# bjing2016/mdgen

Hardware: AMD Instinct MI355X
Metric: sampled MD frames/sec (higher is better)
Workload: dtype bf16; 1 GPU; tetrapeptide_fwdsim_crop4_T1000_B16; batch_per_gpu=16, num_frames=1000, crop=4, euler_steps=49, hipgraph=True, parallelism=batch-sharded x1, no collective

## Files before the change

mdgen_amd/csrc/k_rows.hip:

```cpp
#include "kernels.h"
#include "rows.h"

namespace mdg {

struct MlpPipe {
    f32x16 y[12];
    f32x16 a1[2][2];
    bf16x8 hf[2][4];
    bf16x8 wr[kWRing];
    f32x4 bias;
    float gx[4], gp[4], gq[4];
};

__device__ __forceinline__ void acc_rearm(f32x16& t, int r, float b) {
    float z;
    asm("v_accvgpr_write_b32 %0, %1" : "=a"(z) : "v"(b));
    t[r] = z;
}
constexpr float kGelu3C0 = -2.301208258e+00f, kGelu3C1 = -1.066924557e-01f, kGelu3C2 = 1.000115648e-03f;
template <int ST, bool REARM>
__device__ __forceinline__ void gelu_stage(MlpPipe& m, f32x16 (&a1r)[2], int g, bf16x8 (&hfw)[4]) {
    const int tile = g >> 2, a = g & 3;
    if (ST == 0) {
#pragma unroll
        for (int j = 0; j < 4; ++j) asm("v_accvgpr_read_b32 %0, %1" : "=v"(m.gx[j]) : "a"(a1r[tile][4 * a + j]));
    } else if (ST == 1) {
#pragma unroll
        for (int j = 0; j < 4; ++j) m.gq[j] = m.gx[j] * m.gx[j];
    } else if (ST == 2) {
#pragma unroll
        for (int j = 0; j < 4; ++j) m.gq[j] = fminf(m.gq[j], 64.0f);
    } else if (ST == 3) {
#pragma unroll
        for (int j = 0; j < 4; ++j) m.gp[j] = kGelu3C2 * m.gq[j] + kGelu3C1;
    } else if (ST == 4) {
#pragma unroll
        for (int j = 0; j < 4; ++j) m.gp[j] = m.gp[j] * m.gq[j] + kGelu3C0;
    } else if (ST == 5) {
#pragma unroll
        for (int j = 0; j < 4; ++j) m.gp[j] = m.gx[j] * m.gp[j];
    } else if (ST == 6) {
        m.gp[0] = __builtin_amdgcn_exp2f(m.gp[0]);
        m.gp[1] = __builtin_amdgcn_exp2f(m.gp[1]);
        if (REARM) {
            acc_rearm(a1r[tile], 4 * a + 0, m.bias[0]);
            acc_rearm(a1r[tile], 4 * a + 1, m.bias[1]);
        }
    } else if (ST == 7) {
        m.gp[2] = __builtin_amdgcn_exp2f(m.gp[2]);
        m.gp[3] = __builtin_amdgcn_exp2f(m.gp[3]);
        m.gp[0] = 1.0f + m.gp[0];
        m.gp[1] = 1.0f + m.gp[1];
    } else if (ST == 8) {
        m.gp[0] = __builtin_amdgcn_rcpf(m.gp[0]);
        m.gp[1] = __builtin_amdgcn_rcpf(m.gp[1]);
        m.gp[2] = 1.0f + m.gp[2];
        m.gp[3] = 1.0f + m.gp[3];
    } else if (ST == 9) {
        m.gp[2] = __builtin_amdgcn_rcpf(m.gp[2]);
        m.gp[3] = __builtin_amdgcn_rcpf(m.gp[3]);
        m.gx[0] = m.gx[0] * m.gp[0];
        m.gx[1] = m.gx[1] * m.gp[1];
    } else if (ST == 10) {
        m.gx[2] = m.gx[2] * m.gp[2];
        m.gx[3] = m.gx[3] * m.gp[3];
        if (REARM) {
            acc_rearm(a1r[tile], 4 * a + 2, m.bias[2]);
            acc_rearm(a1r[tile], 4 * a + 3, m.bias[3]);
        }
    } else {
        const int kk = 2 * tile + (a >> 1), e0 = 4 * (a & 1);
        hfw[kk][e0 + 0] = (__bf16)m.gx[0];
        hfw[kk][e0 + 1] = (__bf16)m.gx[1];
        hfw[kk][e0 + 2] = (__bf16)m.gx[2];
        hfw[kk][e0 + 3] = (__bf16)m.gx[3];
    }
}
template <bool REARM, int ST = 0>
__device__ __forceinline__ void gelu_stages_from(MlpPipe& m, f32x16 (&a1r)[2], int g, bf16x8 (&hfw)[4]) {
    gelu_stage<ST, REARM>(m, a1r, g, hfw);
    if constexpr (ST < 11) gelu_stages_from<REARM, ST + 1>(m, a1r, g, hfw);
}
__device__ __forceinline__ void rearm(f32x16 (&a1r)[2], int g, const f32x4& b) {
    const int tile = g >> 2, a = g & 3;
#pragma unroll
    for (int j = 0; j < 4; ++j) acc_rearm(a1r[tile], 4 * a + j, b[j]);
}
__device__ __forceinline__ void arm_chunk(f32x16 (&a1)[2], const float* b1c) {
#pragma unroll
    for (int g = 0; g < 8; ++g) rearm(a1, g, *reinterpret_cast<const f32x4*>(b1c + 32 * (g >> 2) + 8 * (g & 3)));
}

template <class WS, int D0, int STRIDE>
__device__ __forceinline__ void issue_q(const WS& ws, long slot, int q) {
    switch (q / STRIDE) {
        case 0: ws.template issue<D0 + 0>(slot); break;
        case 1: ws.template issue<D0 + 1>(slot); break;
        case 2: ws.template issue<D0 + 2>(slot); break;
        case 3: if constexpr (12 / STRIDE > 3) ws.template issue<D0 + 3>(slot); break;
        case 4: if constexpr (12 / STRIDE > 4) ws.template issue<D0 + 4>(slot); break;
        case 5: if constexpr (12 / STRIDE > 5) ws.template issue<D0 + 5>(slot); break;
        case 6: if constexpr (12 / STRIDE > 6) ws.template issue<D0 + 6>(slot); break;
        case 7: if constexpr (12 / STRIDE > 7) ws.template issue<D0 + 7>(slot); break;
        case 8: if constexpr (12 / STRIDE > 8) ws.template issue<D0 + 8>(slot); break;
        case 9: if constexpr (12 / STRIDE > 9) ws.template issue<D0 + 9>(slot); break;
        case 10: if constexpr (12 / STRIDE > 10) ws.template issue<D0 + 10>(slot); break;
        default: if constexpr (12 / STRIDE > 11) ws.template issue<D0 + 11>(slot); break;
    }
}

template <bool REARM>
__device__ __forceinline__ void gelu_stage_q(MlpPipe& m, f32x16 (&a1r)[2], int g, int q, bf16x8 (&hfw)[4]) {
    switch (q) {
        case 0: gelu_stage<0, REARM>(m, a1r, g, hfw); break;
        case 1: gelu_stage<1, REARM>(m, a1r, g, hfw); break;
        case 2: gelu_stage<2, REARM>(m, a1r, g, hfw); break;
        case 3: gelu_stage<3, REARM>(m, a1r, g, hfw); break;
        case 4: gelu_stage<4, REARM>(m, a1r, g, hfw); break;
        case 5: gelu_stage<5, REARM>(m, a1r, g, hfw); break;
        case 6: gelu_stage<6, REARM>(m, a1r, g, hfw); break;
        case 7: gelu_stage<7, REARM>(m, a1r, g, hfw); break;
        case 8: gelu_stage<8, REARM>(m, a1r, g, hfw); break;
        case 9: gelu_stage<9, REARM>(m, a1r, g, hfw); break;
        case 10: gelu_stage<10, REARM>(m, a1r, g, hfw); break;
        default: gelu_stage<11, REARM>(m, a1r, g, hfw); break;
    }
}

template <int NW, int I0, int KIND, int KI, int GG, bool REARM, int BARVM, bool FILL, int NLOOK = 12, class WS>
__device__ __forceinline__ void pipe_block(MlpPipe& m, const bf16x8 (&xf)[24], f32x16 (&a1w)[2], f32x16 (&a1r)[2],
                                           bf16x8 (&hfw)[4], const bf16x8 (&hfr)[4], const float* b1n,
                                           const unsigned char* ring_lane, const WS& ws, long fill_slot) {
    constexpr int FPW = WS::FPW, DPB = FPW / 2, STRIDE = 12 / DPB;
    if (BARVM >= 0) ring_barrier<BARVM>();
    __builtin_amdgcn_sched_barrier(0);
#pragma unroll
    for (int q = 0; q < 12; ++q) {
        const int I = I0 + q;
        if (FILL && q % STRIDE == 0) issue_q<WS, ((I0 / 12) & 1) * DPB, STRIDE>(ws, fill_slot, q);
        if (q < NLOOK) m.wr[(I + kWPF) % kWRing] = *reinterpret_cast<const bf16x8*>(ring_lane + ((I + kWPF) % kRingFrags) * 1024);
        if (GG >= 0 && REARM && q == 0) m.bias = *reinterpret_cast<const f32x4*>(b1n + 32 * (GG >> 2) + 8 * (GG & 3));
        if (KIND == 0) {
            const int ks = 6 * KI + (q >> 1), tile = q & 1;
            a1w[tile] = __builtin_amdgcn_mfma_f32_32x32x16_bf16(m.wr[I % kWRing], xf[ks], a1w[tile], 0, 0, 0);
        } else {
            m.y[q] = __builtin_amdgcn_mfma_f32_32x32x16_bf16(m.wr[I % kWRing], hfr[KI], m.y[q], 0, 0, 0);
        }
        if (GG >= 0) gelu_stage_q<REARM>(m, a1r, GG, q, hfw);
        __builtin_amdgcn_sched_barrier(0);
    }
}

template <bool REARM>
__device__ __forceinline__ void gelu_group_plain(MlpPipe& m, f32x16 (&a1r)[2], const float* b1n, int g, bf16x8 (&hfw)[4]) {
    if (REARM) m.bias = *reinterpret_cast<const f32x4*>(b1n + 32 * (g >> 2) + 8 * (g & 3));
    gelu_stages_from<REARM>(m, a1r, g, hfw);
}

#define ROWS_STAMP(i)                                  \
    st[i] = __builtin_amdgcn_s_memtime();              \
    __builtin_amdgcn_sched_barrier(0)

template <int NW, bool MODLDS, bool FOLD = false, bool TAIL = false>
__global__ __launch_bounds__(NW * 64, 1) void k_mlp_rows(const MlpRowsParams p) {
    static_assert(!FOLD || MODLDS, "the folded form: one modulation group per launch");
    static_assert(!TAIL || FOLD, "the tail runs on the folded form's accumulators");
    __shared__ __attribute__((aligned(1024))) unsigned char smem[kRingBytes + 8192 + NW * 6144 + (TAIL ? 4096 : 0)];
    using WS = WStream<NW>;
    constexpr int FPW = WS::FPW;
    const int w = __builtin_amdgcn_readfirstlane(wave_id()), lane = lane_id(), hh = lane >> 5, n = lane & 31;
    unsigned long long st[8] = {};
    ROWS_STAMP(0);
    WS ws{p.wstream, lds_addr(smem), (unsigned)lane * 16u, w};
#pragma unroll
    for (int i = 0; i < 6; ++i)
        if (i % NW == w)
            dma_frag<0, true>(reinterpret_cast<const unsigned char*>(p.b1) + i * 1024, (unsigned)lane * 16u,
                              lds_addr(smem) + kRingBytes + i * 1024);
    if (TAIL) {
#pragma unroll
        for (int c = 0; c < 2; ++c)
            if (c % NW == w) {
                const unsigned char* src = reinterpret_cast<const unsigned char*>(p.tail_mod) + c * (kC * 4);
                dma_frag<0, true>(src, (unsigned)lane * 16u, lds_addr(smem) + kRingBytes + 8192 + NW * 6144 + c * 2048);
                dma_frag<1024, false>(src, (unsigned)lane * 16u, lds_addr(smem) + kRingBytes + 8192 + NW * 6144 + c * 2048);
            }
    }
    const long t = ((long)blockIdx.x * NW + w) * 32 + n;
    const int tok = t < p.nrows ? (int)t : -1;
    float* modl = reinterpret_cast<float*>(smem + kRingBytes + 8192 + w * 6144);
    {
        if (MODLDS) {
            const long t0 = ((long)blockIdx.x * NW + w) * 32;
            const unsigned char* mb = reinterpret_cast<const unsigned char*>(p.mm.mod + p.mm.row_off(t0 < p.nrows ? t0 : 0));
            const int chunk[3] = {p.scale_chunk, p.shift_chunk, p.gate_chunk};
#pragma unroll
            for (int c = 0; c < 3; ++c) {
                const unsigned char* src = FOLD && c == 2 ? reinterpret_cast<const unsigned char*>(p.b2g) : mb + (long)chunk[c] * (kC * 4);
                dma_frag<0, true>(src, (unsigned)lane * 16u, lds_addr(modl) + c * 2048);
                dma_frag<1024, false>(src, (unsigned)lane * 16u, lds_addr(modl) + c * 2048);
            }
        }
    }
    ws.issue_slot(0);
    ws.issue_slot(1);
    ws.issue_slot(2);
    float* b1s = reinterpret_cast<float*>(smem + kRingBytes);
    bf16x8 xf[24];
    MlpPipe m;
    const unsigned char* ring_lane = smem + lane * 16;
    if (MODLDS) {
        f32x4 v[48];
        rows_load(p.h, tok, v);
        asm volatile("s_waitcnt vmcnt(0)" ::: "memory");
        if (FOLD) rows_norm_lds_fold(v, tok, modl, modl + 512, modl + 1024, 1e-6f, xf, m.y);
        else rows_norm_lds(v, tok, modl, modl + 512, 1e-6f, xf);
    } else {
        rows_ln(p.h, tok, p.mm, p.shift_chunk, p.scale_chunk, 1e-6f, xf);
    }
    ROWS_STAMP(1);
    if (!FOLD) rows_acc_init(m.y, p.b2);
    const float* b1l = b1s + 4 * hh;
    ring_barrier<FPW>();
#pragma unroll
    for (int i = 0; i < kWPF; ++i) m.wr[i] = *reinterpret_cast<const bf16x8*>(ring_lane + i * 1024);
    arm_chunk(m.a1[0], b1l);
    arm_chunk(m.a1[1], b1l + 64);
    pipe_block<NW, 0, 0, 0, -1, false, -1, true>(m, xf, m.a1[0], m.a1[1], m.hf[0], m.hf[1], b1l, ring_lane, ws, 3);
    pipe_block<NW, 12, 0, 1, -1, false, -1, true>(m, xf, m.a1[0], m.a1[1], m.hf[0], m.hf[1], b1l, ring_lane, ws, 3);
    pipe_block<NW, 24, 0, 2, -1, false, FPW, true>(m, xf, m.a1[0], m.a1[1], m.hf[0], m.hf[1], b1l, ring_lane, ws, 4);
    pipe_block<NW, 36, 0, 3, -1, false, -1, true>(m, xf, m.a1[0], m.a1[1], m.hf[0], m.hf[1], b1l, ring_lane, ws, 4);
    pipe_block<NW, 48, 0, 0, 0, true, FPW, true>(m, xf, m.a1[1], m.a1[0], m.hf[0], m.hf[1], b1l + 128, ring_lane, ws, 5);
    gelu_group_plain<true>(m, m.a1[0], b1l + 128, 1, m.hf[0]);
    pipe_block<NW, 60, 0, 1, 2, true, -1, true>(m, xf, m.a1[1], m.a1[0], m.hf[0], m.hf[1], b1l + 128, ring_lane, ws, 5);
    gelu_group_plain<true>(m, m.a1[0], b1l + 128, 3, m.hf[0]);
    pipe_block<NW, 72, 0, 2, 4, true, FPW, true>(m, xf, m.a1[1], m.a1[0], m.hf[0], m.hf[1], b1l + 128, ring_lane, ws, 6);
    gelu_group_plain<true>(m, m.a1[0], b1l + 128, 5, m.hf[0]);
    pipe_block<NW, 84, 0, 3, 6, true, -1, true>(m, xf, m.a1[1], m.a1[0], m.hf[0], m.hf[1], b1l + 128, ring_lane, ws, 6);
    gelu_group_plain<true>(m, m.a1[0], b1l + 128, 7, m.hf[0]);
    ROWS_STAMP(2);
#pragma unroll 1
    for (int c = 1; c < 23; c += 2) {
        {
            const long s0 = 4 * c;
            const float* bn = b1l + 64 * (c + 2);
            pipe_block<NW, 0, 0, 0, 0, true, FPW, true>(m, xf, m.a1[0], m.a1[1], m.hf[1], m.hf[0], bn, ring_lane, ws, s0 + 3);
            pipe_block<NW, 12, 1, 0, 1, true, -1, true>(m, xf, m.a1[0], m.a1[1], m.hf[1], m.hf[0], bn, ring_lane, ws, s0 + 3);
            pipe_block<NW, 24, 0, 1, 2, true, FPW, true>(m, xf, m.a1[0], m.a1[1], m.hf[1], m.hf[0], bn, ring_lane, ws, s0 + 4);
            pipe_block<NW, 36, 1, 1, 3, true, -1, true>(m, xf, m.a1[0], m.a1[1], m.hf[1], m.hf[0], bn, ring_lane, ws, s0 + 4);
            pipe_block<NW, 48, 0, 2, 4, true, FPW, true>(m, xf, m.a1[0], m.a1[1], m.hf[1], m.hf[0], bn, ring_lane, ws, s0 + 5);
            pipe_block<NW, 60, 1, 2, 5, true, -1, true>(m, xf, m.a1[0], m.a1[1], m.hf[1], m.hf[0], bn, ring_lane, ws, s0 + 5);
            pipe_block<NW, 72, 0, 3, 6, true, FPW, true>(m, xf, m.a1[0], m.a1[1], m.hf[1], m.hf[0], bn, ring_lane, ws, s0 + 6);
            pipe_block<NW, 84, 1, 3, 7, true, -1, true>(m, xf, m.a1[0], m.a1[1], m.hf[1], m.hf[0], bn, ring_lane, ws, s0 + 6);
        }
        {
            const long s0 = 4 * (c + 1);
            const float* bn = b1l + 64 * (c + 3);
            pipe_block<NW, 0, 0, 0, 0, true, FPW, true>(m, xf, m.a1[1], m.a1[0], m.hf[0], m.hf[1], bn, ring_lane, ws, s0 + 3);
            pipe_block<NW, 12, 1, 0, 1, true, -1, true>(m, xf, m.a1[1], m.a1[0], m.hf[0], m.hf[1], bn, ring_lane, ws, s0 + 3);
            pipe_block<NW, 24, 0, 1, 2, true, FPW, true>(m, xf, m.a1[1], m.a1[0], m.hf[0], m.hf[1], bn, ring_lane, ws, s0 + 4);
            pipe_block<NW, 36, 1, 1, 3, true, -1, true>(m, xf, m.a1[1], m.a1[0], m.hf[0], m.hf[1], bn, ring_lane, ws, s0 + 4);
            pipe_block<NW, 48, 0, 2, 4, true, FPW, true>(m, xf, m.a1[1], m.a1[0], m.hf[0], m.hf[1], bn, ring_lane, ws, s0 + 5);
            pipe_block<NW, 60, 1, 2, 5, true, -1, true>(m, xf, m.a1[1], m.a1[0], m.hf[0], m.hf[1], bn, ring_lane, ws, s0 + 5);
            pipe_block<NW, 72, 0, 3, 6, true, FPW, true>(m, xf, m.a1[1], m.a1[0], m.hf[0], m.hf[1], bn, ring_lane, ws, s0 + 6);
            pipe_block<NW, 84, 1, 3, 7, true, -1, true>(m, xf, m.a1[1], m.a1[0], m.hf[0], m.hf[1], bn, ring_lane, ws, s0 + 6);
        }
    }
    ROWS_STAMP(3);
    pipe_block<NW, 0, 1, 0, 0, false, FPW, true>(m, xf, m.a1[0], m.a1[1], m.hf[1], m.hf[0], b1l, ring_lane, ws, 95);
    gelu_group_plain<false>(m, m.a1[1], b1l, 1, m.hf[1]);
    pipe_block<NW, 12, 1, 1, 2, false, -1, true>(m, xf, m.a1[0], m.a1[1], m.hf[1], m.hf[0], b1l, ring_lane, ws, 95);
    gelu_group_plain<false>(m, m.a1[1], b1l, 3, m.hf[1]);
    pipe_block<NW, 24, 1, 2, 4, false, FPW, false>(m, xf, m.a1[0], m.a1[1], m.hf[1], m.hf[0], b1l, ring_lane, ws, 0);
    gelu_group_plain<false>(m, m.a1[1], b1l, 5, m.hf[1]);
    pipe_block<NW, 36, 1, 3, 6, false, -1, false>(m, xf, m.a1[0], m.a1[1], m.hf[1], m.hf[0], b1l, ring_lane, ws, 0);
    gelu_group_plain<false>(m, m.a1[1], b1l, 7, m.hf[1]);
    pipe_block<NW, 48, 1, 0, -1, false, 0, false>(m, xf, m.a1[0], m.a1[1], m.hf[0], m.hf[1], b1l, ring_lane, ws, 0);
    pipe_block<NW, 60, 1, 1, -1, false, -1, false>(m, xf, m.a1[0], m.a1[1], m.hf[0], m.hf[1], b1l, ring_lane, ws, 0);
    pipe_block<NW, 72, 1, 2, -1, false, 0, false>(m, xf, m.a1[0], m.a1[1], m.hf[0], m.hf[1], b1l, ring_lane, ws, 0);
    pipe_block<NW, 84, 1, 3, -1, false, -1, false, 12 - kWPF>(m, xf, m.a1[0], m.a1[1], m.hf[0], m.hf[1], b1l, ring_lane, ws, 0);
    ROWS_STAMP(4);
    if (TAIL) {
        const float* fmod = reinterpret_cast<const float*>(smem + kRingBytes + 8192 + NW * 6144);
        float xnew[16];
        rows_final_tail(m.y, tok, fmod + 512, fmod, p.tail_w, p.tail_b, p.tail_D, p.tail_euler, p.tail_dt, p.tail_x, p.tail_out, xf, xnew);
        ROWS_STAMP(6);
        if (p.emb_base) {
            rows_embed_tail(m.y, tok, xnew, EmbedTail{p.emb_wl_hi, p.emb_wl_lo, p.emb_wc_hi, p.emb_wc_lo, p.emb_base, p.emb_mdelta, p.emb_xcond, p.emb_cmask, p.emb_T, p.emb_L, p.tail_D});
            ROWS_STAMP(7);
            rows_write<0, 12>(m.y, tok, p.h);
        }
    } else if (FOLD) {
        rows_write<0, 12>(m.y, tok, p.h);
    } else if (MODLDS) {
        rows_gate_residual_lds<0, 6>(m.y, tok, modl + 1024, p.h);
        rows_gate_residual_lds<6, 12>(m.y, tok, modl + 1024, p.h);
    } else {
        rows_gate_residual<0, 6>(m.y, tok, p.mm, p.gate_chunk, p.h);
        rows_gate_residual<6, 12>(m.y, tok, p.mm, p.gate_chunk, p.h);
    }
    ROWS_STAMP(5);
    if (p.trace && lane == 0) {
        const long i = ((long)blockIdx.x * NW + w) * 8;
        if (i + 8 <= p.trace_cap) {
#pragma unroll
            for (int k = 0; k < 8; ++k) p.trace[i + k] = st[k];
        }
    }
}

__global__ void k_pack_stream(const float* __restrict__ wsrc, int ld, int which, const int* __restrict__ tab, int nfrag,
                              float scale, int kappa, bf16x8* __restrict__ dst, const int* __restrict__ rowmap) {
    const long i = (long)blockIdx.x * blockDim.x + threadIdx.x;
    if (i >= (long)nfrag * 64) return;
    const int lane = (int)(i & 63), f = (int)(i >> 6);
    const int e = tab[f];
    if ((e >> 16) != which) return;
    const int tile = (e >> 8) & 255, ks = e & 255;
    const int hh = lane >> 5;
    const int row = rowmap ? rowmap[tile * 32 + (lane & 31)] : tile * 32 + (lane & 31);
    bf16x8 v;
#pragma unroll
    for (int j = 0; j < 8; ++j) {
        const int col = kappa == 1 ? 16 * ks + 8 * (j >> 2) + 4 * hh + (j & 3) : 16 * ks + 8 * hh + j;
        v[j] = (__bf16)(wsrc[(long)row * ld + col] * scale);
    }
    dst[i] = v;
}

struct PackFoldParams {
    const float* mod;
    long mod_step_stride;
    int nl;
    int goff[8];
    const float* w2[8];
    const float* b2[8];
    const bf16x8* base[8];
    const int* tab;
    bf16x8* dst;
    float* b2g;
};
__global__ __launch_bounds__(256) void k_pack_fold(const PackFoldParams p) {
    const int sl = blockIdx.y, s = sl / p.nl, l = sl % p.nl;
    const int i = blockIdx.x * 256 + threadIdx.x;
    const int lane = i & 63, f = i >> 6;
    const float* gate = p.mod + (long)s * p.mod_step_stride + p.goff[l];
    if (blockIdx.x == 0)
        for (int c = threadIdx.x; c < kC; c += 256) p.b2g[(size_t)sl * kC + c] = gate[c] * p.b2[l][c];
    const int e = p.tab[f];
    bf16x8 v;
    if ((e >> 16) == 0) {
        v = p.base[l][i];
    } else {
        const int tile = (e >> 8) & 255, ks = e & 255, hh = lane >> 5;
        const int row = tile * 32 + (lane & 31);
        const float g = gate[row];
        const float* wr = p.w2[l] + (size_t)row * kF + 16 * ks + 4 * hh;
        const f32x4 a = *reinterpret_cast<const f32x4*>(wr), b = *reinterpret_cast<const f32x4*>(wr + 8);
#pragma unroll
        for (int j = 0; j < 4; ++j) {
            v[j] = (__bf16)(a[j] * g);
            v[4 + j] = (__bf16)(b[j] * g);
        }
    }
    p.dst[(size_t)sl * (2304 * 64) + i] = v;
}
void launch_pack_fold(const float* mod, long mod_step_stride, int S, int nl, const int* goff, const float* const* w2,
                      const float* const* b2, const bf16x8* const* base, const int* tab, bf16x8* dst, float* b2g, hipStream_t s) {
    PackFoldParams p{};
    p.mod = mod;
    p.mod_step_stride = mod_step_stride;
    p.nl = nl;
    for (int l = 0; l < nl; ++l) {
        p.goff[l] = goff[l];
        p.w2[l] = w2[l];
        p.b2[l] = b2[l];
        p.base[l] = base[l];
    }
    p.tab = tab;
    p.dst = dst;
    p.b2g = b2g;
    hipLaunchKernelGGL(k_pack_fold, dim3(2304 * 64 / 256, (unsigned)(S * nl)), dim3(256), 0, s, p);
}

__global__ void k_sub_f32(const float* __restrict__ a, const float* __restrict__ b, float* __restrict__ dst, int n) {
    const int i = blockIdx.x * 256 + threadIdx.x;
    if (i < n) dst[i] = a[i] - b[i];
}
void launch_sub_f32(const float* a, const float* b, float* dst, int n, hipStream_t s) {
    hipLaunchKernelGGL(k_sub_f32, dim3((n + 255) / 256), dim3(256), 0, s, a, b, dst, n);
}
__global__ __launch_bounds__(96) void k_embed_base(const float* __restrict__ bl, const float* __restrict__ bc, const float* __restrict__ mask_emb,
                                                   const float* __restrict__ pos_embed, const float* __restrict__ ipa_out, int BL, int L,
                                                   float* __restrict__ base) {
    const long row = blockIdx.x;
    const int l = (int)(row % BL) % L, c = threadIdx.x * 4;
    f32x4 v = *reinterpret_cast<const f32x4*>(bl + c);
    const f32x4 a = *reinterpret_cast<const f32x4*>(bc + c), m0 = *reinterpret_cast<const f32x4*>(mask_emb + c),
                ip = *reinterpret_cast<const f32x4*>(ipa_out + row * kC + c);
    f32x4 pe = {0.f, 0.f, 0.f, 0.f};
    if (pos_embed) pe = *reinterpret_cast<const f32x4*>(pos_embed + (size_t)l * kC + c);
#pragma unroll
    for (int k = 0; k < 4; ++k) v[k] = ((v[k] + a[k]) + m0[k]) + (pe[k] + ip[k]);
    *reinterpret_cast<f32x4*>(base + row * kC + c) = v;
}
void launch_embed_base(const float* bl, const float* bc, const float* mask_emb, const float* pos_embed, const float* ipa_out, int S,
                       int BL, int L, float* base, hipStream_t s) {
    hipLaunchKernelGGL(k_embed_base, dim3((unsigned)((long)S * BL)), dim3(96), 0, s, bl, bc, mask_emb, pos_embed, ipa_out, BL, L, base);
}

void launch_pack_stream(const float* w, int ld, int which, const int* tab, int nfrag, float scale, int kappa, bf16x8* dst,
                        hipStream_t s, const int* rowmap) {
    const long total = (long)nfrag * 64;
    hipLaunchKernelGGL(k_pack_stream, dim3((unsigned)((total + 255) / 256)), dim3(256), 0, s, w, ld, which, tab, nfrag, scale, kappa, dst,
                       rowmap);
}

void launch_mlp_rows(const MlpRowsParams& p, MlpRowsForm form, hipStream_t s) {
    constexpr int NW = 4;
    const bool uni = p.mm.tokens_per_group % 32 == 0 || (p.mm.step_stride == 0 && p.mm.group_stride == 0);
    const long tiles = (p.nrows + 31) / 32;
    const dim3 g((unsigned)((tiles + NW - 1) / NW)), b(NW * 64);
    const bool fold = form != MlpRowsForm::Plain, tail = form == MlpRowsForm::FoldFinal || form == MlpRowsForm::FoldFinalEmbed;
    if (fold != (p.b2g != nullptr) || tail != (p.tail_w != nullptr) || (form == MlpRowsForm::FoldFinalEmbed) != (p.emb_base != nullptr) ||
        (fold && (p.mm.step_stride != 0 || p.mm.group_stride != 0))) {
        g_k32_launch_error = "launch_mlp_rows: the form and the fold / tail / embedding operands disagree";
        return;
    }
    switch (form) {
    case MlpRowsForm::FoldFinal:
    case MlpRowsForm::FoldFinalEmbed: hipLaunchKernelGGL((k_mlp_rows<NW, true, true, true>), g, b, 0, s, p); return;
    case MlpRowsForm::Fold: hipLaunchKernelGGL((k_mlp_rows<NW, true, true>), g, b, 0, s, p); return;
    case MlpRowsForm::Plain:
        if (uni) hipLaunchKernelGGL((k_mlp_rows<NW, true>), g, b, 0, s, p);
        else hipLaunchKernelGGL((k_mlp_rows<NW, false>), g, b, 0, s, p);
        return;
    }
}

}
```

mdgen_amd/csrc/rows.h:

```cpp
#pragma once
#include "common.h"

namespace mdg {

constexpr int kSlotFrags = 24;
constexpr int kSlotBytes = kSlotFrags * 1024;
constexpr int kRingSlots = 4;
constexpr int kRingFrags = kRingSlots * kSlotFrags;
constexpr int kRingBytes = kRingSlots * kSlotBytes;
constexpr int kWPF = 5;
constexpr int kWRing = kWPF + 1;

typedef __attribute__((address_space(3))) unsigned char lds_u8;
__device__ __forceinline__ unsigned lds_addr(const void* p) { return (unsigned)(uintptr_t)(const lds_u8*)p; }

__device__ __forceinline__ float half_sum2(float x) {
    const auto r = __builtin_amdgcn_permlane32_swap(__float_as_uint(x), __float_as_uint(x), false, false);
    return __uint_as_float(r[0]) + __uint_as_float(r[1]);
}

__device__ __forceinline__ float acc_zero() {
    float z;
    asm volatile("v_accvgpr_write_b32 %0, 0" : "=a"(z));
    return z;
}

template <int OFF, bool SETM0>
__device__ __forceinline__ void dma_frag(const unsigned char* src, unsigned voff, unsigned lds_dst) {
    static_assert(OFF >= 0 && OFF < 4096, "13-bit signed instruction offset");
    if (SETM0)
        asm volatile("s_mov_b32 m0, %2\n\ts_nop 0\n\tglobal_load_lds_dwordx4 %0, %1 offset:%3" ::"v"(voff), "s"(src), "s"(lds_dst), "n"(OFF) : "memory");
    else
        asm volatile("global_load_lds_dwordx4 %0, %1 offset:%2" ::"v"(voff), "s"(src), "n"(OFF) : "memory");
}

template <int VM>
__device__ __forceinline__ void ring_barrier() {
    asm volatile("s_waitcnt vmcnt(%0) lgkmcnt(0)\n\ts_barrier" ::"n"(VM) : "memory");
}

template <int NW>
struct WStream {
    static constexpr int FPW = kSlotFrags / NW;
    const unsigned char* src;
    unsigned ring;
    unsigned voff;
    int w;
    template <int D>
    __device__ __forceinline__ void issue(long slot) const {
        const int f = w * FPW + (D & ~3);
        const unsigned char* base = src + slot * kSlotBytes;
        dma_frag<(D & 3) * 1024, (D & 3) == 0>(base + f * 1024, voff, ring + ((unsigned)slot & 3u) * kSlotBytes + f * 1024);
    }
    template <int D0 = 0>
    __device__ __forceinline__ void issue_slot(long slot) const {
        issue<D0>(slot);
        if constexpr (D0 + 1 < FPW) issue_slot<D0 + 1>(slot);
    }
};

template <int I>
__device__ __forceinline__ bf16x8 ring_frag(const unsigned char* ring_lane) {
    return *reinterpret_cast<const bf16x8*>(ring_lane + (I % kRingFrags) * 1024);
}

__device__ __forceinline__ void rows_load(const float* __restrict__ x, int tok, f32x4 (&v)[48]) {
    const int hh = lane_id() >> 5;
    const unsigned tokc = tok < 0 ? 0u : (unsigned)tok;
    const unsigned char* xb = reinterpret_cast<const unsigned char*>(x);
    const unsigned off = tokc * (unsigned)(kC * 4) + (unsigned)hh * 16u;
#pragma unroll
    for (int i = 0; i < 48; ++i) v[i] = *reinterpret_cast<const f32x4*>(xb + off + 32u * i);
}
__device__ __forceinline__ void rows_norm(const f32x4 (&v)[48], int tok, const ModMap mm, int shift_chunk, int scale_chunk,
                                          float eps, bf16x8 (&xf)[24]) {
    const int hh = lane_id() >> 5;
    const unsigned tokc = tok < 0 ? 0u : (unsigned)tok;
    const unsigned mo = tok < 0 ? 0u : (unsigned)mm.row_off(tokc);
    const unsigned char* mb = reinterpret_cast<const unsigned char*>(mm.mod);
    const unsigned osc = (mo + (unsigned)(scale_chunk * kC)) * 4u + (unsigned)hh * 16u;
    const unsigned osh = (mo + (unsigned)(shift_chunk * kC)) * 4u + (unsigned)hh * 16u;
    float s = 0.f;
#pragma unroll
    for (int i = 0; i < 48; ++i) s += (v[i][0] + v[i][1]) + (v[i][2] + v[i][3]);
    const float mean = half_sum2(s) * (1.0f / kC);
    float q = 0.f;
#pragma unroll
    for (int i = 0; i < 48; ++i) {
#pragma unroll
        for (int j = 0; j < 4; ++j) {
            const float d = v[i][j] - mean;
            q += d * d;
        }
    }
    const float rstd = tok < 0 ? 0.f : 1.0f / sqrtf(half_sum2(q) * (1.0f / kC) + eps);
    const float live = tok < 0 ? 0.f : 1.f;
    float mean2 = mean;
    asm volatile("" : "+v"(mean2));
    constexpr int kModPF = 2;
    f32x4 sc[kModPF + 1][2], sh[kModPF + 1][2];
#pragma unroll
    for (int ks = 0; ks < kModPF; ++ks)
#pragma unroll
        for (int h2 = 0; h2 < 2; ++h2) {
            sc[ks][h2] = *reinterpret_cast<const f32x4*>(mb + osc + 32u * (2 * ks + h2));
            sh[ks][h2] = *reinterpret_cast<const f32x4*>(mb + osh + 32u * (2 * ks + h2));
        }
    __builtin_amdgcn_sched_barrier(0);
#pragma unroll
    for (int ks = 0; ks < 24; ++ks) {
        if (ks + kModPF < 24) {
#pragma unroll
            for (int h2 = 0; h2 < 2; ++h2) {
                sc[(ks + kModPF) % (kModPF + 1)][h2] = *reinterpret_cast<const f32x4*>(mb + osc + 32u * (2 * (ks + kModPF) + h2));
                sh[(ks + kModPF) % (kModPF + 1)][h2] = *reinterpret_cast<const f32x4*>(mb + osh + 32u * (2 * (ks + kModPF) + h2));
            }
        }
        uint32_t u[4];
#pragma unroll
        for (int h2 = 0; h2 < 2; ++h2) {
            const f32x4 c = sc[ks % (kModPF + 1)][h2], d = sh[ks % (kModPF + 1)][h2];
            const f32x4 a = v[2 * ks + h2];
            const float y0 = (a[0] - mean2) * (rstd * c[0] + rstd) + live * d[0];
            const float y1 = (a[1] - mean2) * (rstd * c[1] + rstd) + live * d[1];
            const float y2 = (a[2] - mean2) * (rstd * c[2] + rstd) + live * d[2];
            const float y3 = (a[3] - mean2) * (rstd * c[3] + rstd) + live * d[3];
            u[2 * h2] = pack_bf16(y0, y1);
            u[2 * h2 + 1] = pack_bf16(y2, y3);
        }
        u32x4 t = {u[0], u[1], u[2], u[3]};
        asm volatile("" : "+v"(t));
        xf[ks] = __builtin_bit_cast(bf16x8, t);
        __builtin_amdgcn_sched_barrier(0);
    }
}

__device__ __forceinline__ void rows_norm_lds(const f32x4 (&v)[48], int tok, const float* sc, const float* sh, float eps,
                                              bf16x8 (&xf)[24]) {
    const int hh = lane_id() >> 5;
    float s = 0.f;
#pragma unroll
    for (int i = 0; i < 48; ++i) s += (v[i][0] + v[i][1]) + (v[i][2] + v[i][3]);
    const float mean = half_sum2(s) * (1.0f / kC);
    float q = 0.f;
#pragma unroll
    for (int i = 0; i < 48; ++i) {
#pragma unroll
        for (int j = 0; j < 4; ++j) {
            const float d = v[i][j] - mean;
            q += d * d;
        }
    }
    const float rstd = tok < 0 ? 0.f : 1.0f / sqrtf(half_sum2(q) * (1.0f / kC) + eps);
    const float live = tok < 0 ? 0.f : 1.f;
    float mean2 = mean;
    asm volatile("" : "+v"(mean2));
    const f32x4* scp = reinterpret_cast<const f32x4*>(sc + 4 * hh);
    const f32x4* shp = reinterpret_cast<const f32x4*>(sh + 4 * hh);
#pragma unroll
    for (int ks = 0; ks < 24; ++ks) {
        uint32_t u[4];
#pragma unroll
        for (int h2 = 0; h2 < 2; ++h2) {
            const f32x4 c = scp[2 * (2 * ks + h2)], d = shp[2 * (2 * ks + h2)];
            const f32x4 a = v[2 * ks + h2];
            const float y0 = (a[0] - mean2) * (rstd * c[0] + rstd) + live * d[0];
            const float y1 = (a[1] - mean2) * (rstd * c[1] + rstd) + live * d[1];
            const float y2 = (a[2] - mean2) * (rstd * c[2] + rstd) + live * d[2];
            const float y3 = (a[3] - mean2) * (rstd * c[3] + rstd) + live * d[3];
            u[2 * h2] = pack_bf16(y0, y1);
            u[2 * h2 + 1] = pack_bf16(y2, y3);
        }
        xf[ks] = __builtin_bit_cast(bf16x8, u32x4{u[0], u[1], u[2], u[3]});
    }
}

__device__ __forceinline__ void rows_norm_lds_fold(const f32x4 (&v)[48], int tok, const float* sc, const float* sh, const float* b2g,
                                                   float eps, bf16x8 (&xf)[24], f32x16 (&y)[12]) {
    const int hh = lane_id() >> 5;
    float s = 0.f;
#pragma unroll
    for (int i = 0; i < 48; ++i) s += (v[i][0] + v[i][1]) + (v[i][2] + v[i][3]);
    const float mean = half_sum2(s) * (1.0f / kC);
    float q = 0.f;
#pragma unroll
    for (int i = 0; i < 48; ++i) {
#pragma unroll
        for (int j = 0; j < 4; ++j) {
            const float d = v[i][j] - mean;
            q += d * d;
        }
    }
    const float rstd = tok < 0 ? 0.f : 1.0f / sqrtf(half_sum2(q) * (1.0f / kC) + eps);
    const float live = tok < 0 ? 0.f : 1.f;
    float mean2 = mean;
    asm volatile("" : "+v"(mean2));
    const f32x4* scp = reinterpret_cast<const f32x4*>(sc + 4 * hh);
    const f32x4* shp = reinterpret_cast<const f32x4*>(sh + 4 * hh);
    const f32x4* bgp = reinterpret_cast<const f32x4*>(b2g + 4 * hh);
#pragma unroll
    for (int ks = 0; ks < 24; ++ks) {
        uint32_t u[4];
#pragma unroll
        for (int h2 = 0; h2 < 2; ++h2) {
            const int i = 2 * ks + h2;
            const f32x4 c = scp[2 * i], d = shp[2 * i], b = bgp[2 * i];
            const f32x4 a = v[i];
            const float y0 = (a[0] - mean2) * (rstd * c[0] + rstd) + live * d[0];
            const float y1 = (a[1] - mean2) * (rstd * c[1] + rstd) + live * d[1];
            const float y2 = (a[2] - mean2) * (rstd * c[2] + rstd) + live * d[2];
            const float y3 = (a[3] - mean2) * (rstd * c[3] + rstd) + live * d[3];
            u[2 * h2] = pack_bf16(y0, y1);
            u[2 * h2 + 1] = pack_bf16(y2, y3);
#pragma unroll
            for (int j = 0; j < 4; ++j) y[i >> 2][4 * (i & 3) + j] = a[j] + b[j];
        }
        xf[ks] = __builtin_bit_cast(bf16x8, u32x4{u[0], u[1], u[2], u[3]});
    }
}

template <int FT0, int FT1>
__device__ __forceinline__ void rows_write(const f32x16 (&y)[12], int tok, float* __restrict__ h) {
    const int hh = lane_id() >> 5;
    const unsigned tokc = tok < 0 ? 0u : (unsigned)tok;
    unsigned char* hb = reinterpret_cast<unsigned char*>(h);
    const unsigned off = tokc * (unsigned)(kC * 4) + (unsigned)hh * 16u;
    if (tok >= 0) {
#pragma unroll
        for (int i = FT0 * 4; i < FT1 * 4; ++i) {
            const int ft = i >> 2, a = i & 3;
            const f32x4 o = {y[ft][4 * a], y[ft][4 * a + 1], y[ft][4 * a + 2], y[ft][4 * a + 3]};
            *reinterpret_cast<f32x4*>(hb + off + 32u * (unsigned)i) = o;
        }
    }
}

__device__ __forceinline__ void rows_final_tail(const f32x16 (&y)[12], int tok, const float* sc, const float* sh,
                                                const bf16x8* __restrict__ wfin, const float* __restrict__ bfin, int D, int euler,
                                                float dt, float* __restrict__ x, float* __restrict__ out, bf16x8 (&xf)[24],
                                                float (&xnew)[16]) {
    const int lane = lane_id(), hh = lane >> 5;
    const unsigned tokc = tok < 0 ? 0u : (unsigned)tok;
    f32x4 b4[4];
#pragma unroll
    for (int a = 0; a < 4; ++a) b4[a] = *reinterpret_cast<const f32x4*>(bfin + 8 * a + 4 * hh);
    float xv[16];
    float* xp = (euler ? x : out) + (size_t)tokc * (unsigned)D;
#pragma unroll
    for (int r = 0; r < 16; ++r) {
        const int f = 8 * (r >> 2) + 4 * hh + (r & 3);
        xv[r] = euler ? xp[f < D ? f : 0] : 0.f;
    }
    f32x4 v[48];
#pragma unroll
    for (int i = 0; i < 48; ++i)
#pragma unroll
        for (int j = 0; j < 4; ++j) asm("v_accvgpr_read_b32 %0, %1" : "=v"(v[i][j]) : "a"(y[i >> 2][4 * (i & 3) + j]));
    rows_norm_lds(v, tok, sc, sh, 1e-6f, xf);
    __builtin_amdgcn_sched_barrier(0);
    bf16x8 wf[24];
#pragma unroll
    for (int ks = 0; ks < 24; ++ks) wf[ks] = wfin[ks * 64 + lane];
    f32x16 acc;
#pragma unroll
    for (int r = 0; r < 16; ++r) acc[r] = b4[r >> 2][r & 3];
#pragma unroll
    for (int ks = 0; ks < 24; ++ks) acc = __builtin_amdgcn_mfma_f32_32x32x16_bf16(wf[ks], xf[ks], acc, 0, 0, 0);
    const float s = euler ? dt : 1.0f;
#pragma unroll
    for (int r = 0; r < 16; ++r) {
        const int f = 8 * (r >> 2) + 4 * hh + (r & 3);
        xnew[r] = f < D ? xv[r] + s * acc[r] : 0.f;
        if (tok >= 0 && f < D) xp[f] = xnew[r];
    }
}

__device__ __forceinline__ void rows_embed_gemm_split(f32x16 (&y)[12], const bf16x8* __restrict__ whi, const bf16x8* __restrict__ wlo,
                                                      const float (&xv)[16]) {
    const int lane = lane_id();
    bf16x8 xh[2], xl[2];
#pragma unroll
    for (int s = 0; s < 2; ++s)
#pragma unroll
        for (int j = 0; j < 8; ++j) {
            const __bf16 h = (__bf16)xv[8 * s + j];
            xh[s][j] = h;
            xl[s][j] = (__bf16)(xv[8 * s + j] - (float)h);
        }
    bf16x8 wh[2][2], wl[2][2];
#pragma unroll
    for (int s = 0; s < 2; ++s) {
        wh[0][s] = whi[s * 64 + lane];
        wl[0][s] = wlo[s * 64 + lane];
    }
    __builtin_amdgcn_sched_barrier(0);
#pragma unroll
    for (int ft = 0; ft < 12; ++ft) {
        if (ft + 1 < 12) {
#pragma unroll
            for (int s = 0; s < 2; ++s) {
                wh[(ft + 1) & 1][s] = whi[((ft + 1) * 2 + s) * 64 + lane];
                wl[(ft + 1) & 1][s] = wlo[((ft + 1) * 2 + s) * 64 + lane];
            }
        }
        __builtin_amdgcn_sched_barrier(0);
#pragma unroll
        for (int s = 0; s < 2; ++s) {
            y[ft] = __builtin_amdgcn_mfma_f32_32x32x16_bf16(wl[ft & 1][s], xh[s], y[ft], 0, 0, 0);
            y[ft] = __builtin_amdgcn_mfma_f32_32x32x16_bf16(wh[ft & 1][s], xl[s], y[ft], 0, 0, 0);
        }
#pragma unroll
        for (int s = 0; s < 2; ++s) y[ft] = __builtin_amdgcn_mfma_f32_32x32x16_bf16(wh[ft & 1][s], xh[s], y[ft], 0, 0, 0);
        __builtin_amdgcn_sched_barrier(0);
    }
}
struct EmbedTail {
    const bf16x8 *wl_hi, *wl_lo, *wc_hi, *wc_lo;
    const float* base;
    const float* mdelta;
    const float* x_cond;
    const int64_t* x_cond_mask;
    int T, L, D;
};
__device__ __forceinline__ void rows_embed_tail(f32x16 (&y)[12], int tok, const float (&xnew)[16], const EmbedTail e) {
    const int lane = lane_id(), hh = lane >> 5;
    const unsigned tokc = tok < 0 ? 0u : (unsigned)tok;
    const unsigned row = (tokc / (unsigned)(e.T * e.L)) * (unsigned)e.L + tokc % (unsigned)e.L;
    const unsigned char* bb = reinterpret_cast<const unsigned char*>(e.base) + (size_t)row * (kC * 4) + hh * 16;
#pragma unroll
    for (int i = 0; i < 48; ++i) {
        const f32x4 b = *reinterpret_cast<const f32x4*>(bb + 32u * i);
#pragma unroll
        for (int j = 0; j < 4; ++j) y[i >> 2][4 * (i & 3) + j] = b[j];
    }
    float xc[16];
    const float* cp = e.x_cond + (size_t)tokc * (unsigned)e.D;
#pragma unroll
    for (int r = 0; r < 16; ++r) {
        const int f = 8 * (r >> 2) + 4 * hh + (r & 3);
        const float v = cp[f < e.D ? f : 0];
        xc[r] = f < e.D && tok >= 0 ? v : 0.f;
    }
    const bool cm = tok >= 0 && e.x_cond_mask[tokc] != 0;
    rows_embed_gemm_split(y, e.wl_hi, e.wl_lo, xnew);
    bool anyc = false;
#pragma unroll
    for (int r = 0; r < 16; ++r) anyc |= xc[r] != 0.f;
    if (__builtin_amdgcn_ballot_w64(anyc) != 0) {
        rows_embed_gemm_split(y, e.wc_hi, e.wc_lo, xc);
    }
    if (__builtin_amdgcn_ballot_w64(cm) != 0) {
        const unsigned char* mb = reinterpret_cast<const unsigned char*>(e.mdelta) + hh * 16;
        const float sel = cm ? 1.f : 0.f;
#pragma unroll
        for (int i = 0; i < 48; ++i) {
            const f32x4 d = *reinterpret_cast<const f32x4*>(mb + 32u * i);
#pragma unroll
            for (int j = 0; j < 4; ++j) y[i >> 2][4 * (i & 3) + j] += sel * d[j];
        }
    }
}

__device__ __forceinline__ void rows_ln(const float* __restrict__ x, int tok, const ModMap mm, int shift_chunk,
                                        int scale_chunk, float eps, bf16x8 (&xf)[24]) {
    f32x4 v[48];
    rows_load(x, tok, v);
    rows_norm(v, tok, mm, shift_chunk, scale_chunk, eps, xf);
}

__device__ __forceinline__ void rows_acc_init(f32x16 (&y)[12], const float* __restrict__ bias) {
    const unsigned char* bb = reinterpret_cast<const unsigned char*>(bias) + (lane_id() >> 5) * 16;
#pragma unroll
    for (int ft = 0; ft < 12; ++ft)
#pragma unroll
        for (int a = 0; a < 4; ++a) {
            const f32x4 b = *reinterpret_cast<const f32x4*>(bb + 32u * (4 * ft + a));
#pragma unroll
            for (int j = 0; j < 4; ++j) y[ft][4 * a + j] = b[j];
        }
}

template <int FT0, int FT1>
__device__ __forceinline__ void rows_gate_residual(const f32x16 (&y)[12], int tok, const ModMap mm, int gate_chunk,
                                                   float* __restrict__ h) {
    const int hh = lane_id() >> 5;
    const unsigned tokc = tok < 0 ? 0u : (unsigned)tok;
    unsigned char* hb = reinterpret_cast<unsigned char*>(h);
    const unsigned off = tokc * (unsigned)(kC * 4) + (unsigned)hh * 16u;
    const unsigned mo = tok < 0 ? 0u : (unsigned)mm.row_off(tokc);
    const unsigned char* mb = reinterpret_cast<const unsigned char*>(mm.mod);
    const unsigned og = (mo + (unsigned)(gate_chunk * kC)) * 4u + (unsigned)hh * 16u;
    constexpr int NV = (FT1 - FT0) * 4;
    f32x4 hv[NV], g[NV];
#pragma unroll
    for (int i = 0; i < NV; ++i) {
        const unsigned fo = 32u * (unsigned)(FT0 * 4 + i);
        hv[i] = *reinterpret_cast<const f32x4*>(hb + off + fo);
        g[i] = *reinterpret_cast<const f32x4*>(mb + og + fo);
    }
#pragma unroll
    for (int i = 0; i < NV; ++i) {
        const int ft = FT0 + (i >> 2), a = i & 3;
        f32x4 o = hv[i];
#pragma unroll
        for (int j = 0; j < 4; ++j) o[j] += g[i][j] * y[ft][4 * a + j];
        if (tok >= 0) *reinterpret_cast<f32x4*>(hb + off + 32u * (unsigned)(FT0 * 4 + i)) = o;
    }
}

template <int FT0, int FT1>
__device__ __forceinline__ void rows_gate_residual_lds(const f32x16 (&y)[12], int tok, const float* gate, float* __restrict__ h) {
    const int hh = lane_id() >> 5;
    const unsigned tokc = tok < 0 ? 0u : (unsigned)tok;
    unsigned char* hb = reinterpret_cast<unsigned char*>(h);
    const unsigned off = tokc * (unsigned)(kC * 4) + (unsigned)hh * 16u;
    const f32x4* gp = reinterpret_cast<const f32x4*>(gate + 4 * hh);
    constexpr int NV = (FT1 - FT0) * 4;
    f32x4 hv[NV];
#pragma unroll
    for (int i = 0; i < NV; ++i) hv[i] = *reinterpret_cast<const f32x4*>(hb + off + 32u * (unsigned)(FT0 * 4 + i));
#pragma unroll
    for (int i = 0; i < NV; ++i) {
        const int ft = FT0 + (i >> 2), a = i & 3;
        const f32x4 g = gp[2 * (FT0 * 4 + i)];
        f32x4 o = hv[i];
#pragma unroll
        for (int j = 0; j < 4; ++j) o[j] += g[j] * y[ft][4 * a + j];
        if (tok >= 0) *reinterpret_cast<f32x4*>(hb + off + 32u * (unsigned)(FT0 * 4 + i)) = o;
    }
}

}
```

Baseline: 126,900 frames/s.

## Prefetch tail weights and embedding base rows into LDS during final MLP blocks

In the fused tail kernel, the last four MLP pipe blocks now also DMA the final-layer weights and embedding weights into the freed ring slots. The per-sample embedding base rows are staged into LDS midway through the MLP. rows_final_tail and rows_embed_tail then read these operands from LDS instead of global memory, hiding the global load latency behind MFMA work. A waitcnt and barrier are added before writing xnew, and a fallback to global loads remains when a wave's tokens span samples not staged. This raises LDS usage and adds synchronization, and correctness depends on the ring slots no longer being needed.

New measurement: 127,400 frames/s, median of 6. Within noise of the previous version (+0.4%).

```diff
diff --git a/mdgen_amd/csrc/k_rows.hip b/mdgen_amd/csrc/k_rows.hip
--- a/mdgen_amd/csrc/k_rows.hip
+++ b/mdgen_amd/csrc/k_rows.hip
@@ -272,21 +272,52 @@
     pipe_block<NW, 12, 1, 1, 2, false, -1, true>(m, xf, m.a1[0], m.a1[1], m.hf[1], m.hf[0], b1l, ring_lane, ws, 95);
     gelu_group_plain<false>(m, m.a1[1], b1l, 3, m.hf[1]);
     pipe_block<NW, 24, 1, 2, 4, false, FPW, false>(m, xf, m.a1[0], m.a1[1], m.hf[1], m.hf[0], b1l, ring_lane, ws, 0);
+    const unsigned emb_tl = (unsigned)(p.emb_T * p.emb_L);
+    const int emb_s0 = TAIL ? (int)((blockIdx.x * (unsigned)(NW * 32)) / (emb_tl ? emb_tl : 1u)) : -1;
+    if (TAIL) {
+        const unsigned char* bsrc = p.emb_base ? reinterpret_cast<const unsigned char*>(p.emb_base) + (size_t)emb_s0 * p.emb_L * (kC * 4)
+                                               : reinterpret_cast<const unsigned char*>(p.tail_w);
+#pragma unroll
+        for (int d = 0; d < kBaseLdsBytes / 1024 / NW; ++d) {
+            const int piece = w * (kBaseLdsBytes / 1024 / NW) + d;
+            const unsigned u = (unsigned)piece * 64u + (unsigned)lane;
+            unsigned row = u / (unsigned)kBaseLdsUnits, ch = u % (unsigned)kBaseLdsUnits;
+            row = (int)row < p.emb_L ? row : 0u;
+            ch = ch < (unsigned)(kC / 4) ? ch : 0u;
+            dma_frag<0, true>(bsrc, row * (unsigned)(kC * 4) + ch * 16u, lds_addr(smem) + kRingBytes + piece * 1024);
+        }
+    }
     gelu_group_plain<false>(m, m.a1[1], b1l, 5, m.hf[1]);
     pipe_block<NW, 36, 1, 3, 6, false, -1, false>(m, xf, m.a1[0], m.a1[1], m.hf[1], m.hf[0], b1l, ring_lane, ws, 0);
     gelu_group_plain<false>(m, m.a1[1], b1l, 7, m.hf[1]);
-    pipe_block<NW, 48, 1, 0, -1, false, 0, false>(m, xf, m.a1[0], m.a1[1], m.hf[0], m.hf[1], b1l, ring_lane, ws, 0);
-    pipe_block<NW, 60, 1, 1, -1, false, -1, false>(m, xf, m.a1[0], m.a1[1], m.hf[0], m.hf[1], b1l, ring_lane, ws, 0);
-    pipe_block<NW, 72, 1, 2, -1, false, 0, false>(m, xf, m.a1[0], m.a1[1], m.hf[0], m.hf[1], b1l, ring_lane, ws, 0);
-    pipe_block<NW, 84, 1, 3, -1, false, -1, false, 12 - kWPF>(m, xf, m.a1[0], m.a1[1], m.hf[0], m.hf[1], b1l, ring_lane, ws, 0);
+    if constexpr (TAIL) {
+        const unsigned char* wfin_g = reinterpret_cast<const unsigned char*>(p.tail_w);
+        const TailFill<NW> tfin{wfin_g, ws.ring, ws.voff, w};
+        const TailFill2<NW> temb{{p.emb_base ? reinterpret_cast<const unsigned char*>(p.emb_wl_hi) : wfin_g, ws.ring, ws.voff, w},
+                                 {p.emb_base ? reinterpret_cast<const unsigned char*>(p.emb_wl_lo) : wfin_g, ws.ring, ws.voff, w}};
+        pipe_block<NW, 48, 1, 0, -1, false, 0, true>(m, xf, m.a1[0], m.a1[1], m.hf[0], m.hf[1], b1l, ring_lane, tfin, 0);
+        pipe_block<NW, 60, 1, 1, -1, false, -1, true>(m, xf, m.a1[0], m.a1[1], m.hf[0], m.hf[1], b1l, ring_lane, tfin, 0);
+        pipe_block<NW, 72, 1, 2, -1, false, 0, true>(m, xf, m.a1[0], m.a1[1], m.hf[0], m.hf[1], b1l, ring_lane, temb, 1);
+        pipe_block<NW, 84, 1, 3, -1, false, -1, true, 12 - kWPF>(m, xf, m.a1[0], m.a1[1], m.hf[0], m.hf[1], b1l, ring_lane, temb, 1);
+    } else {
+        pipe_block<NW, 48, 1, 0, -1, false, 0, false>(m, xf, m.a1[0], m.a1[1], m.hf[0], m.hf[1], b1l, ring_lane, ws, 0);
+        pipe_block<NW, 60, 1, 1, -1, false, -1, false>(m, xf, m.a1[0], m.a1[1], m.hf[0], m.hf[1], b1l, ring_lane, ws, 0);
+        pipe_block<NW, 72, 1, 2, -1, false, 0, false>(m, xf, m.a1[0], m.a1[1], m.hf[0], m.hf[1], b1l, ring_lane, ws, 0);
+        pipe_block<NW, 84, 1, 3, -1, false, -1, false, 12 - kWPF>(m, xf, m.a1[0], m.a1[1], m.hf[0], m.hf[1], b1l, ring_lane, ws, 0);
+    }
     ROWS_STAMP(4);
     if (TAIL) {
         const float* fmod = reinterpret_cast<const float*>(smem + kRingBytes + 8192 + NW * 6144);
         float xnew[16];
-        rows_final_tail(m.y, tok, fmod + 512, fmod, p.tail_w, p.tail_b, p.tail_D, p.tail_euler, p.tail_dt, p.tail_x, p.tail_out, xf, xnew);
+        rows_final_tail(m.y, tok, fmod + 512, fmod, reinterpret_cast<const bf16x8*>(smem), p.tail_b, p.tail_D, p.tail_euler, p.tail_dt,
+                        p.tail_x, p.tail_out, xf, xnew);
         ROWS_STAMP(6);
         if (p.emb_base) {
-            rows_embed_tail(m.y, tok, xnew, EmbedTail{p.emb_wl_hi, p.emb_wl_lo, p.emb_wc_hi, p.emb_wc_lo, p.emb_base, p.emb_mdelta, p.emb_xcond, p.emb_cmask, p.emb_T, p.emb_L, p.tail_D});
+            rows_embed_tail(m.y, tok, xnew,
+                            EmbedTail{reinterpret_cast<const bf16x8*>(smem + kSlotBytes), reinterpret_cast<const bf16x8*>(smem + 2 * kSlotBytes),
+                                      p.emb_wc_hi, p.emb_wc_lo, p.emb_base, (const lds_u8*)(smem + kRingBytes),
+                                      p.emb_L * kBaseLdsStride <= kBaseLdsBytes ? emb_s0 : -1, p.emb_mdelta, p.emb_xcond, p.emb_cmask,
+                                      p.emb_T, p.emb_L, p.tail_D});
             ROWS_STAMP(7);
             rows_write<0, 12>(m.y, tok, p.h);
         }
diff --git a/mdgen_amd/csrc/rows.h b/mdgen_amd/csrc/rows.h
--- a/mdgen_amd/csrc/rows.h
+++ b/mdgen_amd/csrc/rows.h
@@ -59,6 +59,33 @@
     }
 };
 
+template <int NW>
+struct TailFill {
+    static constexpr int FPW = kSlotFrags / NW;
+    const unsigned char* src;
+    unsigned ring, voff;
+    int w;
+    template <int D>
+    __device__ __forceinline__ void issue(long pos) const {
+        const int f = w * FPW + D;
+        dma_frag<0, true>(src + f * 1024, voff, ring + (unsigned)pos * kSlotBytes + f * 1024);
+    }
+};
+template <int NW>
+struct TailFill2 {
+    static constexpr int FPW = 2 * TailFill<NW>::FPW;
+    TailFill<NW> a, b;
+    template <int D>
+    __device__ __forceinline__ void issue(long pos) const {
+        if constexpr (D < FPW / 2) a.template issue<D>(pos);
+        else b.template issue<D - FPW / 2>(pos + 1);
+    }
+};
+
+constexpr int kBaseLdsStride = kC * 4 + 32;
+constexpr int kBaseLdsUnits = kBaseLdsStride / 16;
+constexpr int kBaseLdsBytes = 8192;
+
 template <int I>
 __device__ __forceinline__ bf16x8 ring_frag(const unsigned char* ring_lane) {
     return *reinterpret_cast<const bf16x8*>(ring_lane + (I % kRingFrags) * 1024);
@@ -271,6 +298,11 @@
     for (int r = 0; r < 16; ++r) {
         const int f = 8 * (r >> 2) + 4 * hh + (r & 3);
         xnew[r] = f < D ? xv[r] + s * acc[r] : 0.f;
+    }
+    asm volatile("s_waitcnt vmcnt(0)\n\ts_barrier" ::: "memory");
+#pragma unroll
+    for (int r = 0; r < 16; ++r) {
+        const int f = 8 * (r >> 2) + 4 * hh + (r & 3);
         if (tok >= 0 && f < D) xp[f] = xnew[r];
     }
 }
@@ -317,6 +349,8 @@
 struct EmbedTail {
     const bf16x8 *wl_hi, *wl_lo, *wc_hi, *wc_lo;
     const float* base;
+    const lds_u8* base_lds;
+    int lds_sample;
     const float* mdelta;
     const float* x_cond;
     const int64_t* x_cond_mask;
@@ -325,14 +359,6 @@
 __device__ __forceinline__ void rows_embed_tail(f32x16 (&y)[12], int tok, const float (&xnew)[16], const EmbedTail e) {
     const int lane = lane_id(), hh = lane >> 5;
     const unsigned tokc = tok < 0 ? 0u : (unsigned)tok;
-    const unsigned row = (tokc / (unsigned)(e.T * e.L)) * (unsigned)e.L + tokc % (unsigned)e.L;
-    const unsigned char* bb = reinterpret_cast<const unsigned char*>(e.base) + (size_t)row * (kC * 4) + hh * 16;
-#pragma unroll
-    for (int i = 0; i < 48; ++i) {
-        const f32x4 b = *reinterpret_cast<const f32x4*>(bb + 32u * i);
-#pragma unroll
-        for (int j = 0; j < 4; ++j) y[i >> 2][4 * (i & 3) + j] = b[j];
-    }
     float xc[16];
     const float* cp = e.x_cond + (size_t)tokc * (unsigned)e.D;
 #pragma unroll
@@ -341,7 +367,29 @@
         const float v = cp[f < e.D ? f : 0];
         xc[r] = f < e.D && tok >= 0 ? v : 0.f;
     }
-    const bool cm = tok >= 0 && e.x_cond_mask[tokc] != 0;
+    const int64_t cmv = e.x_cond_mask[tokc];
+    const bool cm = tok >= 0 && cmv != 0;
+    const unsigned smp = tokc / (unsigned)(e.T * e.L), l = tokc % (unsigned)e.L;
+    const bool staged = tok < 0 || (int)smp == e.lds_sample;
+    if (__builtin_amdgcn_ballot_w64(!staged) == 0) {
+        typedef __attribute__((address_space(3))) const f32x4 lds_f32x4;
+        const lds_u8* bl = e.base_lds + l * (unsigned)kBaseLdsStride + hh * 16;
+#pragma unroll
+        for (int i = 0; i < 48; ++i) {
+            const f32x4 b = *reinterpret_cast<lds_f32x4*>(bl + 32u * i);
+#pragma unroll
+            for (int j = 0; j < 4; ++j) y[i >> 2][4 * (i & 3) + j] = b[j];
+        }
+    } else {
+        const unsigned row = smp * (unsigned)e.L + l;
+        const unsigned char* bb = reinterpret_cast<const unsigned char*>(e.base) + (size_t)row * (kC * 4) + hh * 16;
+#pragma unroll
+        for (int i = 0; i < 48; ++i) {
+            const f32x4 b = *reinterpret_cast<const f32x4*>(bb + 32u * i);
+#pragma unroll
+            for (int j = 0; j < 4; ++j) y[i >> 2][4 * (i & 3) + j] = b[j];
+        }
+    }
     rows_embed_gemm_split(y, e.wl_hi, e.wl_lo, xnew);
     bool anyc = false;
 #pragma unroll
```
